# baker-laboratory/NA-MPNN

Hardware: AMD Instinct MI355X
Metric: residues/sec (enc+dec fwd), N~1000 K=48 h=128; seq-recovery vs CPU ref (higher is better)
Workload: dtype f32; 1 GPU; cfg2: B=1 x N=1000 residues per rank, K=48, H=128, 3 enc + 3 dec layers, per-edge GEMMs fp32, seeded random-init weights, independent complexes per rank; precision=fp32, global_batch=1, seq_len=1000, parallelism=replicas x1

## Files before the change

### na_mpnn_amd/csrc/namp.hip

```cpp
#include "../../include/namp.h"
#include "namp_kernels.h"
#include <atomic>
#include "namp_bf16s32.h"
#include "namp_bf16p.h"
#include "namp_node_w.h"
#include "namp_order.h"
#include "namp_attach.h"

#include <cstdarg>
#include <cstdlib>
#include <cstring>
#include <initializer_list>
#include <cstdio>
#include <mutex>
#include <vector>

namespace {

thread_local char g_err[512] = "";

int fail(int code, const char* fmt, ...) {
  va_list ap;
  va_start(ap, fmt);
  vsnprintf(g_err, sizeof(g_err), fmt, ap);
// ... 321 lines not shown
  if (nproj < 0 || nproj > 8 || (nproj > 0 && !proj)) return fail(NAMP_EINVAL, "%s: nproj=%d must be in [0,8]", fn, nproj);
  for (int i = 0; i < nproj; ++i) {
    if (!proj[i].img || !proj[i].out) return fail(NAMP_EINVAL, "%s: proj[%d] has a null image / output", fn, i);
    if (!aligned16(proj[i].img) || !aligned16(proj[i].out) || !aligned16(proj[i].bias) || !aligned16(proj[i].tok))
      return fail(NAMP_EINVAL, "%s: proj[%d] pointers must be 16-byte aligned", fn, i);
    if (proj[i].tok && !S) return fail(NAMP_EINVAL, "%s: proj[%d].tok given but S is null", fn, i);
  }
  return NAMP_OK;
}

struct Out16Req { __bf16* p[8]; int n; bool honoured; };
thread_local Out16Req* g_out16 = nullptr;
thread_local bool g_residue_x1 = false;

int launch_node_linear(const float* X, const int32_t* S, int G_out, int G_src, int N,
                       const NampProj* proj, int nproj, const NampProj* pre, hipStream_t s, bool x3 = false, unsigned* zero = nullptr) {
  NodeLinearArgs a;
  a.X = X; a.S = S; a.G_out = G_out; a.G_src = G_src; a.N = N; a.nproj = nproj; a.zero = zero;
  a.pre.img = pre ? pre->img : nullptr; a.pre.bias = pre ? pre->bias : nullptr;
  a.pre.tok = nullptr; a.pre.out = pre ? pre->out : nullptr;
  for (int i = 0; i < 8; ++i) {
    const NampProj& p = proj[i < nproj ? i : 0];
    a.p[i].img = p.img; a.p[i].bias = p.bias; a.p[i].tok = p.tok; a.p[i].out = p.out;
    a.out16[i] = (g_out16 && i < nproj && i < g_out16->n) ? g_out16->p[i] : nullptr;
    if (a.out16[i]) a.p[i].out = nullptr;
  }
  if (g_out16) g_out16->honoured = true;
  const int units = ((G_out + 15) / 16) * nproj;
  if (x3 && G_out >= 4096 && (g_bf16p.load(std::memory_order_relaxed) & 8) && ensure_attributes() == NAMP_OK) {
    if (g_residue_x1) hipLaunchKernelGGL(node_linear_w_kernel<2>, dim3((G_out + NODEW_ROWS - 1) / NODEW_ROWS), dim3(NODEW_THREADS), NODEW_LDS, s, a);
    else hipLaunchKernelGGL(node_linear_w_kernel<1>, dim3((G_out + NODEW_ROWS - 1) / NODEW_ROWS), dim3(NODEW_THREADS), NODEW_LDS, s, a);
    return NAMP_OK;
  }
  if (x3 && g_residue_x1) hipLaunchKernelGGL(node_linear_kernel<2>, dim3((units + 3) / 4), dim3(256), 0, s, a);
  else if (x3) hipLaunchKernelGGL(node_linear_kernel<1>, dim3((units + 3) / 4), dim3(256), 0, s, a);
  else hipLaunchKernelGGL(node_linear_kernel<0>, dim3((units + 3) / 4), dim3(256), 0, s, a);
  return NAMP_OK;
}

int launch_node_update(const float* ln1_g, const float* ln1_b, const float* Win_img, const float* b_in,
                       const float* Wout_img, const float* b_out, const float* ln2_g, const float* ln2_b,
                       const float* hV, const float* partial, const float* m3_img, const float* m3_b, const int32_t* mask,
                       float* hV_out, const NampProj* proj, int nproj, const int32_t* S, int G, int TPN, hipStream_t s,
                       bool x3 = false) {
  int rc = ensure_attributes();
  if (rc) return rc;
  NodeUpdateArgs a;
  fill_tail(a.t, ln1_g, ln1_b, Win_img, b_in, Wout_img, b_out, ln2_g, ln2_b, hV, mask, hV_out, proj, nproj, S);
  a.t.m3_img = partial ? m3_img : nullptr; a.t.m3_b = m3_b;
  a.partial = partial; a.G = G; a.TPN = TPN;
  const bool multi = x3 || G >= 32 * 2 * device_cus();
  for (int i = 0; i < 8; ++i) {
    a.out16[i] = (multi && g_out16 && i < nproj && i < g_out16->n) ? g_out16->p[i] : nullptr;
    if (a.out16[i]) a.t.p[i].out = nullptr;
  }
  if (multi && g_out16) g_out16->honoured = true;
  if (x3 && g_residue_x1 && a.t.m3_img && !a.t.head_w && nproj <= 4 && G >= 2048 && (g_bf16p.load(std::memory_order_relaxed) & 8))
    hipLaunchKernelGGL(node_update_w_kernel<false>, dim3((G + NODEW_ROWS - 1) / NODEW_ROWS), dim3(NODEW_THREADS), NODEW_LDS, s, a);
  else if (x3 && !g_residue_x1 && a.t.m3_img && !a.t.head_w && nproj <= 4 && G >= 2048 && (g_bf16p.load(std::memory_order_relaxed) & 8))
    hipLaunchKernelGGL(node_update_w_kernel<true>, dim3((G + NODEW_ROWS - 1) / NODEW_ROWS), dim3(NODEW_THREADS), NODEW_LDS, s, a);
  else if (x3 && g_residue_x1)
    hipLaunchKernelGGL((node_update_multi_kernel<2, 2>), dim3((G + 31) / 32), dim3(512), NODE_MULTI_LDS_X3(2), s, a);
  else if (x3)
    hipLaunchKernelGGL((node_update_multi_kernel<2, 1>), dim3((G + 31) / 32), dim3(512), NODE_MULTI_LDS_X3(2), s, a);
  else if (G >= 32 * 2 * device_cus())
    hipLaunchKernelGGL((node_update_multi_kernel<2, 0>), dim3((G + 31) / 32), dim3(512), NODE_MULTI_LDS(2), s, a);
// ... 1756 lines not shown
```

### na_mpnn_amd/csrc/namp_kernels.h

```cpp
#pragma once
#include "namp_device.h"
#ifndef NAMP_MAX_LAYERS
#define NAMP_MAX_LAYERS 8
#endif

static __global__ void pack_image_kernel(const float* __restrict__ W, int ld, int col0, int OUT, int IN,
                                  float* __restrict__ img) {
  const int total = OUT * IN;
  for (int e = blockIdx.x * blockDim.x + threadIdx.x; e < total; e += gridDim.x * blockDim.x) {
    const int r = e & 3, lane = (e >> 2) & 63, t = e >> 8;
    const int ntn = OUT >> 4;
    const int tn = t % ntn, tk = t / ntn;
    const int n = 16 * tn + (lane & 15), k = 16 * tk + 4 * (lane >> 4) + r;
    img[e] = W[(size_t)n * ld + col0 + k];
  }
}

static __global__ void pack_image_bf16_kernel(const float* __restrict__ W, int ld, int col0, __bf16* __restrict__ img) {
  const int e = blockIdx.x * blockDim.x + threadIdx.x;
  if (e >= 128 * 128) return;
  const int j = e & 7, lane = (e >> 3) & 63, tn = (e >> 9) & 7, s = e >> 12;
  const int n = 16 * tn + (lane & 15), k = 32 * s + 16 * (j >> 2) + 4 * (lane >> 4) + (j & 3);
  img[e] = (__bf16)W[(size_t)n * ld + col0 + k];
}
// ... 109 lines not shown
    out[e] = (c < C1) ? nbrs[row * C1 + c] : nodes[((row / NK) * N + idx[row]) * C2 + (c - C1)];
  }
}

struct ProjDesc {
  const float* img;
  const float* bias;
  const float* tok;
  float* out;
};

struct NodeTail {
  const float* hV;
  const int32_t* mask;
  const float* ln1_g; const float* ln1_b;
  const float* Win_img;
  const float* b_in;
  const float* Wout_img;
  const float* b_out;
  const float* ln2_g; const float* ln2_b;
  float* hV_out;
  const int32_t* S;
  const float* m3_img;
  const float* m3_b;
  const float* head_w;
  const float* head_b;
  float* log_probs;
  float* logits;
  int vocab;
  int nproj;
  ProjDesc p[8];
};

__device__ __forceinline__ void tail_head_row(const NodeTail& a, const float* ybase, const int sc, const int orow,
                                              const int lane) {
  float z = -INFINITY;
  if (lane < a.vocab) {
    const float* w = a.head_w + (long)lane * NAMP_H;
    float s0 = 0.f, s1 = 0.f, s2 = 0.f, s3 = 0.f;
#pragma unroll 8
    for (int c = 0; c < NAMP_H; c += 4) {
      const f4 wv = *(const f4*)(w + c);
      s0 = fmaf(wv.x, ybase[(c + 0) * sc], s0); s1 = fmaf(wv.y, ybase[(c + 1) * sc], s1);
      s2 = fmaf(wv.z, ybase[(c + 2) * sc], s2); s3 = fmaf(wv.w, ybase[(c + 3) * sc], s3);
    }
    z = (s0 + s1) + (s2 + s3) + a.head_b[lane];
  }
  float mx = z;
#pragma unroll
  for (int o = 1; o < 64; o <<= 1) mx = fmaxf(mx, __shfl_xor(mx, o));
  float e = (lane < a.vocab) ? expf(z - mx) : 0.f;
#pragma unroll
  for (int o = 1; o < 64; o <<= 1) e += __shfl_xor(e, o);
  if (lane < a.vocab) {
    a.log_probs[(long)orow * a.vocab + lane] = (z - mx) - logf(e);
    if (a.logits) a.logits[(long)orow * a.vocab + lane] = z;
  }
}

#define FFN_LD 132
#define NODE_TAIL_LDS ((16 + 16 + 8 * 16) * FFN_LD * 4)

template <bool DEEP>
__device__ __forceinline__ void node_tail(const NodeTail& a, f4 (&x)[8], const float wsum_m, const int row0, const int nrows, const int G,
                                          float* lds, const int tid, const int wave, const int nwaves, const int lane) {
  float* xs = lds;
// ... 251 lines not shown
    f4 v = c0[nb] + c1[nb];
#pragma unroll
    for (int c = 0; c < 4; ++c) { v[c] += __shfl_xor(v[c], 16); v[c] += __shfl_xor(v[c], 32); }
    o[nb] = v;
  }
}

#define TAIL4_AHEAD 3
template <class FragFn>
__device__ __forceinline__ void tail4_request1(f4 (&wf)[8], const int u, const int lane, FragFn frag) {
#pragma unroll
  for (int tk = 0; tk < 8; ++tk) wf[tk] = frag(u, tk)[lane];
}
template <class FragFn>
__device__ __forceinline__ void tail4_request(f4 (&wf)[TAIL4_AHEAD][8], const int u0, const int total, const int step, const int lane, FragFn frag) {
#pragma unroll
  for (int t = 0; t < TAIL4_AHEAD; ++t) {
    const int u = u0 + t * step;
    tail4_request1(wf[t], u < total ? u : u0, lane, frag);
  }
}
template <class FragFn, class BodyFn, class NextFn>
__device__ __forceinline__ void tail4_phase(f4 (&wf)[TAIL4_AHEAD][8], const int u0, const int total, const int step, const int lane, FragFn frag,
                                            BodyFn body, NextFn next) {
#pragma unroll
  for (int t = 0; t < TAIL4_AHEAD; ++t) {
    const int u = u0 + t * step;
    if (u < total) body(u, wf[t]);
    next(t);
  }
  tail_units<false>(u0 + TAIL4_AHEAD * step, total, step, lane, frag, body);
}

template <int R, typename RowFn, bool SC1, bool M3, bool PF, bool AH>
__device__ __forceinline__ void node_tail_mfma4(const NodeTail& a, f4 (&x)[8], const float wsum_m, const RowFn orow, float* lds,
                                                const int tid, const int wave, const int nwaves, const int lane) {
  static_assert(R == 4 || R == 8, "node_tail_mfma4: 4 or 8 rows");
  constexpr int NB = R / 4;
  constexpr bool AHEAD = AH && !PF && R == 4;
  float* xB = lds;
  float* hB = xB + 128 * R;
  float* oP = hB + 512 * R;
  float* yT = oP + 4 * 128 * R;
  float* red = yT + 128 * R;
  float* yB = red + 64;
  const int m = lane & 15, g = lane >> 4;
  const int cb = (lane >> 2) & 3, j = lane & 3;
  const bool st_lane = lane < 16;
  const auto win_frag = [&](const int u, const int tk) { return (const f4*)a.Win_img + (tk * 32 + u) * 64; };
  const auto wout_frag = [&](const int u, const int tk) { return (const f4*)a.Wout_img + ((8 * (u >> 3) + tk) * 8 + (u & 7)) * 64; };

  f4 wa[AHEAD ? TAIL4_AHEAD : 1][8];
  float bin_a[TAIL4_AHEAD] = {0.f, 0.f, 0.f};
  if constexpr (AHEAD) {
    tail4_request(wa, wave, 32, nwaves, lane, win_frag);
#pragma unroll
    for (int t = 0; t < TAIL4_AHEAD; ++t) {
      const int u = wave + t * nwaves;
      bin_a[t] = a.b_in[16 * (u < 32 ? u : wave) + 4 * cb + g];
    }
  }
  if (M3 && a.m3_img) {
    if (wave == 0 && m < R) {
#pragma unroll
      for (int t = 0; t < 8; ++t) *(f4*)(xB + (m >> 2) * 512 + t * 64 + g * 16 + (m & 3) * 4) = x[t];
      if (g == 0) red[m] = wsum_m;
    }
    __syncthreads();
    {
      f4 xr[NB][8];
      tail4_x<NB>(xr, xB, lane);
      tail_units<PF>(wave, 8, nwaves, lane,
                     [&](const int u, const int tk) { return (const f4*)a.m3_img + (tk * 8 + u) * 64; },
                     [&](const int u, const f4 (&wf)[8]) {
                       f4 o[NB];
                       tail4_unit<NB>(o, wf, xr);
                       if (st_lane) {
                         const f4 b = *(const f4*)(a.m3_b + 16 * u + 4 * cb);
#pragma unroll
                         for (int nb = 0; nb < NB; ++nb) *(f4*)(oP + (4 * nb + j) * NAMP_H + 16 * u + 4 * cb) = o[nb] + b * red[4 * nb + j];
                       }
                     });
    }
    __syncthreads();
    const int mr = m < R ? m : 0;
    int hr = orow(mr);
    if (hr < 0) hr = orow(0) < 0 ? 0 : orow(0);
    const float* hsrc = a.hV + (long)hr * NAMP_H + 4 * g;
#pragma unroll
    for (int t = 0; t < 8; ++t) x[t] = *(const f4*)(hsrc + 16 * t) + *(const f4*)(oP + mr * NAMP_H + 16 * t + 4 * g);
  }

  layernorm_row_T(x, a.ln1_g, a.ln1_b, g);
  if (wave == 0 && m < R) {
#pragma unroll
    for (int t = 0; t < 8; ++t) *(f4*)(xB + (m >> 2) * 512 + t * 64 + g * 16 + (m & 3) * 4) = x[t];
  }
  __syncthreads();
  {
    f4 xr[NB][8];
    tail4_x<NB>(xr, xB, lane);
    const auto body = [&](const int u, const f4 (&wf)[8]) {
      f4 o[NB];
      tail4_unit<NB>(o, wf, xr);
      const int t_ = AHEAD ? (u - wave) / nwaves : 0;
      const float b = (AHEAD && t_ < TAIL4_AHEAD) ? (t_ == 0 ? bin_a[0] : t_ == 1 ? bin_a[1] : bin_a[2]) : a.b_in[16 * u + 4 * cb + g];
#pragma unroll
      for (int nb = 0; nb < NB; ++nb) {
        const float v = g == 0 ? o[nb].x : g == 1 ? o[nb].y : g == 2 ? o[nb].z : o[nb].w;
        hB[((u >> 3) * NB + nb) * 512 + (u & 7) * 64 + cb * 16 + j * 4 + g] = gelu_erf(v + b);
      }
    };
    if constexpr (AHEAD)
      tail4_phase(wa, wave, 32, nwaves, lane, win_frag, body, [&](const int t) {
        const int u = wave + t * nwaves;
        tail4_request1(wa[t], u < 32 ? u : wave, lane, wout_frag);
      });
    else tail_units<PF>(wave, 32, nwaves, lane, win_frag, body);
  }
  __syncthreads();
  {
    const auto body = [&](const int u, const f4 (&wf)[8]) {
      const int tn = u & 7, q = u >> 3;
      f4 xr[NB][8];
      tail4_x<NB>(xr, hB + q * NB * 512, lane);
      f4 o[NB];
      tail4_unit<NB>(o, wf, xr);
      if (st_lane) {
#pragma unroll
        for (int nb = 0; nb < NB; ++nb) *(f4*)(oP + (q * R + 4 * nb + j) * NAMP_H + 16 * tn + 4 * cb) = o[nb];
      }
    };
    if constexpr (AHEAD)
      tail4_phase(wa, wave, 32, nwaves, lane, wout_frag, body, [&](const int pi) {
        if (pi < a.nproj) {
          const int tn = ((wave - pi * 8) % nwaves + nwaves) % nwaves;
          const f4* img = (const f4*)(pi == 0 ? a.p[0].img : pi == 1 ? a.p[1].img : a.p[2].img) + ((tn < 8 ? tn : 0)) * 64 + lane;
#pragma unroll
          for (int tk = 0; tk < 8; ++tk) wa[pi][tk] = img[tk * 8 * 64];
        }
      });
    else tail_units<PF>(wave, 32, nwaves, lane, wout_frag, body);
  }
  __syncthreads();
  const int n_ = tid >> 7, c_ = tid & 127;
  const bool ln_thr = tid < 128 * R;
  const int boff = ln_thr ? (n_ >> 2) * 512 + tail4_off(c_, n_ & 3) : 0;
  float v = 0.f;
  if (ln_thr) {
    v = xB[boff] + a.b_out[c_];
#pragma unroll
    for (int q = 0; q < 4; ++q) v += oP[(q * R + n_) * NAMP_H + c_];
    float s = v;
#pragma unroll
    for (int o = 1; o < 64; o <<= 1) s += __shfl_xor(s, o);
    if (lane == 0) red[wave] = s;
  }
  __syncthreads();
  float d = 0.f;
  if (ln_thr) {
    const float mean = (red[2 * n_] + red[2 * n_ + 1]) * (1.0f / 128.0f);
    d = v - mean;
    float q = d * d;
#pragma unroll
    for (int o = 1; o < 64; o <<= 1) q += __shfl_xor(q, o);
    if (lane == 0) red[32 + wave] = q;
  }
  __syncthreads();
  if (ln_thr) {
    const float rstd = rsqrtf((red[32 + 2 * n_] + red[32 + 2 * n_ + 1]) * (1.0f / 128.0f) + 1e-5f);
    const int orw = orow(n_);
    const float mk = (a.mask && orw >= 0) ? (float)a.mask[orw] : 1.0f;
    const float y = (d * rstd * a.ln2_g[c_] + a.ln2_b[c_]) * mk;
    yT[c_ * R + n_] = y;
    yB[boff] = y;
    if (orw >= 0) st_out<SC1>(a.hV_out + (long)orw * NAMP_H + c_, y);
  }
  if (a.nproj == 0 && !a.head_w) return;
  __syncthreads();
  if (a.head_w) {
    for (int n = wave; n < R; n += nwaves) {
      const int orw = orow(n);
      if (orw >= 0) tail_head_row(a, yT + n, R, orw, lane);
    }
  }
  f4 xr[NB][8];
  tail4_x<NB>(xr, yB, lane);
  int orw[NB];
#pragma unroll
  for (int nb = 0; nb < NB; ++nb) orw[nb] = orow(4 * nb + j);
  auto proj_out = [&](const f4 (&o)[NB], const float* bias, const float* tok, float* out, const int tn) {
    if (!st_lane) return;
    const int c = 16 * tn + 4 * cb;
    const f4 b = bias ? *(const f4*)(bias + c) : (f4){0.f, 0.f, 0.f, 0.f};
#pragma unroll
    for (int nb = 0; nb < NB; ++nb) {
      if (orw[nb] < 0) continue;
      f4 r = o[nb] + b;
      if (tok) r += *(const f4*)(tok + (long)a.S[orw[nb]] * NAMP_H + c);
      float* dst = out + (long)orw[nb] * NAMP_H + c;
      if (SC1) { st_out<true>(dst, r.x); st_out<true>(dst + 1, r.y); st_out<true>(dst + 2, r.z); st_out<true>(dst + 3, r.w); }
      else *(f4*)dst = r;
    }
  };
  if constexpr (PF) {
    tail_units<true>(wave, 8 * (a.nproj < 2 ? a.nproj : 2), nwaves, lane,
                     [&](const int v, const int tk) { return (const f4*)((v >> 3) ? a.p[1].img : a.p[0].img) + (tk * 8 + (v & 7)) * 64; },
                     [&](const int v, const f4 (&wf)[8]) {
                       const bool second = (v >> 3) != 0;
                       f4 o[NB];
                       tail4_unit<NB>(o, wf, xr);
                       proj_out(o, second ? a.p[1].bias : a.p[0].bias, second ? a.p[1].tok : a.p[0].tok, second ? a.p[1].out : a.p[0].out, v & 7);
                     });
    return;
  }
#pragma unroll
  for (int pi = 0; pi < 8; ++pi) {
    if (pi >= a.nproj) break;
    const ProjDesc pd = a.p[pi];
    bool first = AHEAD && pi < TAIL4_AHEAD;
#pragma unroll 1
    for (int tn = ((wave - pi * 8) % nwaves + nwaves) % nwaves; tn < 8; tn += nwaves) {
      f4 o[NB];
      if (first) {
        tail4_unit<NB>(o, wa[pi < TAIL4_AHEAD ? pi : 0], xr);
      } else {
        f4 wf[8];
#pragma unroll
        for (int tk = 0; tk < 8; ++tk) wf[tk] = ((const f4*)pd.img)[(tk * 8 + tn) * 64 + lane];
        tail4_unit<NB>(o, wf, xr);
      }
      first = false;
      proj_out(o, pd.bias, pd.tok, pd.out, tn);
    }
  }
}

template <int R, typename RowFn, bool SC1 = false, bool M3 = true, bool PF = false, bool AH = false>
__device__ __forceinline__ void node_tail_rows(const NodeTail& a, f4 (&x)[8], const float wsum_m, const RowFn orow, float* lds,
                                               const int tid, const int wave, const int nwaves, const int lane) {
#ifndef NAMP_TAIL_VALU
  node_tail_mfma4<R, RowFn, SC1, M3, PF, AH>(a, x, wsum_m, orow, lds, tid, wave, nwaves, lane);
  return;
#endif
  float* xT = lds;
  float* hT = xT + 128 * R;
  float* oP = hT + 512 * R;
  float* yT = oP + 4 * 128 * R;
  float* red = yT + 128 * R;
  const int m = lane & 15, g = lane >> 4;

  if (M3 && a.m3_img) {
    if (wave == 0 && m < R) {
#pragma unroll
      for (int t = 0; t < 8; ++t) {
        xT[(16 * t + 4 * g + 0) * R + m] = x[t].x; xT[(16 * t + 4 * g + 1) * R + m] = x[t].y;
        xT[(16 * t + 4 * g + 2) * R + m] = x[t].z; xT[(16 * t + 4 * g + 3) * R + m] = x[t].w;
      }
      if (g == 0) red[m] = wsum_m;
    }
    __syncthreads();
#pragma unroll 1
    for (int tn = wave; tn < 8; tn += nwaves) {
      f4 wf[8];
#pragma unroll
      for (int tk = 0; tk < 8; ++tk) wf[tk] = ((const f4*)a.m3_img)[(tk * 8 + tn) * 64 + lane];
      float acc[R];
#pragma unroll
      for (int n = 0; n < R; ++n) acc[n] = 0.f;
      rows_fma<R>(acc, wf, xT, g);
#pragma unroll
      for (int n = 0; n < R; ++n) acc[n] = xg_sum(acc[n]);
      if (g == 0) {
        const float b = a.m3_b[16 * tn + m];
#pragma unroll
// ... 285 lines not shown
}

struct EdgeArgs {
  const float* hE;
  float* hE_out;
  const int32_t* E_idx;
  const int32_t* mask;
  const int32_t* mask_attend;
  const int32_t* rank;
  const float* Pa;
  const float* Pj0;
  const float* Pj1;
  const float* W1_img;
  const float* W2_img;
  const float* W3_img;
  const float* b1;
  const float* b2;
  const float* b3;
  const float* ln_g;
  const float* ln_b;
  const float* ePa; const float* ePj;
  const float* eW1_img; const float* eW2_img; const float* eW3_img;
  const float* eb2; const float* eb3;
  uint32_t drop_thresh, drop_seed; float drop_scale;
  const __bf16* hE16; __bf16* hE16_out;
  const __bf16* Pa16; const __bf16* Pj016; const __bf16* Pj116;
  float* partial;
  NodeTail tail;
  int G;
  int G_enc;
  int N, K, TPN;
};

#define EDGE_TAIL_LDS (2 * NAMP_IMG_BYTES + 12 * NAMP_H * 4 + 64 + 2048)

enum { PRE_NONE = 0, PRE_EMBED = 1, PRE_EDGE = 3 };
enum { PREC_F32 = 0, PREC_BF16 = 1, PREC_X3 = 2 };
template <int MODE, int TAIL, int PREC, int PRE, int PERSIST, class Args>
__device__ __forceinline__ void edge_stage(const Args& a, f4 (&x)[8], char* smem) {
  f4 l2pf0 = (f4){0.f, 0.f, 0.f, 0.f}, l2pf1 = l2pf0;
  constexpr bool BF16 = (PREC == PREC_BF16);
  constexpr bool X3 = (PREC == PREC_X3);
  static_assert(PRE == PRE_NONE || (!BF16 && TAIL != 0 && (MODE == MODE_ENC_MSG || MODE == MODE_DEC_MSG)), "PRE: fp32-class message + tail only");
  constexpr bool FUSE = (PRE == PRE_EDGE);
  constexpr bool MSG = (MODE == MODE_ENC_MSG || MODE == MODE_DEC_MSG);
  constexpr bool M3_LDS = MSG && !BF16 && (TAIL == 4 || TAIL == 8);
  char* buf0 = smem;
  char* buf1 = smem + NAMP_IMG_BYTES;
  const int tid = threadIdx.x;
  const int lane = tid & 63;
  const int wave = __builtin_amdgcn_readfirstlane(tid >> 6);
  const int nwaves = blockDim.x >> 6;

  const int m = lane & 15, g = lane >> 4;
  const int npw = nwaves / a.TPN;
  const int node_l = wave / a.TPN, kt = wave - node_l * a.TPN;
  const int bid = xcd_block_index(blockIdx.x, gridDim.x);
  int node = bid * npw + node_l;
  const bool wave_active = (node_l < npw) && (node < a.G);
  if (!wave_active) node = 0;
  const int b_dec = node / a.N;
  const int i_loc = node - b_dec * a.N;
  const int node_enc = (MODE == MODE_DEC_MSG) ? ((b_dec % (a.G_enc / a.N)) * a.N + i_loc) : node;
  const int k = 16 * kt + m;
  const bool valid = wave_active && (k < a.K);
  const long erow = (long)node_enc * a.K + (valid ? k : 0);

// ... 16 lines not shown
    const int j_loc = a.E_idx[erow];
    const int j = node_enc - i_loc + j_loc;
    const float* pa = a.ePa + (long)node_enc * NAMP_H + 4 * g;
    const float* pj = a.ePj + (long)j * NAMP_H + 4 * g;
#pragma unroll
    for (int t = 0; t < 8; ++t) { acc[t] = *(const f4*)(pa + 16 * t); pjv[t] = *(const f4*)(pj + 16 * t); }
  } else {
    const int j_loc = a.E_idx[erow];
    const float* pj;
    if (MODE == MODE_DEC_MSG) {
      const int j_dec = b_dec * a.N + j_loc;
      const bool bw = a.rank[j_dec] < a.rank[node];
      pj = bw ? (a.Pj0 + (long)j_dec * NAMP_H) : (a.Pj1 + (long)(node_enc - i_loc + j_loc) * NAMP_H);
      w_row = valid ? (1.0f / 30.0f) : 0.f;
    } else {
      const int j = node - i_loc + j_loc;
      pj = a.Pj0 + (long)j * NAMP_H;
      if (MODE == MODE_ENC_MSG) {
        int ma;
        if (a.mask_attend) ma = a.mask_attend[erow];
        else ma = a.mask ? (a.mask[node] * a.mask[j]) : 1;
        w_row = valid ? ((float)ma * (1.0f / 30.0f)) : 0.f;
      }
    }
    const float* pa = a.Pa + (long)node * NAMP_H + 4 * g;
    pj += 4 * g;
#pragma unroll
    for (int t = 0; t < 8; ++t) { acc[t] = *(const f4*)(pa + 16 * t); pjv[t] = *(const f4*)(pj + 16 * t); }
  }

  const f4* w0 = (const f4*)buf0 + lane;
  const f4* w1 = (const f4*)buf1 + lane;

  if (BF16) {
    const bf8* bw = (const bf8*)smem + lane;
    dma_to_lds(smem, a.W1_img, 32, wave, nwaves, lane);
    if (MODE != MODE_EMBED) dma_to_lds(smem + NAMP_BIMG_BYTES, a.W2_img, 32, wave, nwaves, lane);
    if (MODE == MODE_ENC_EDGE) dma_to_lds(smem + 2 * NAMP_BIMG_BYTES, a.W3_img, 32, wave, nwaves, lane);
    wait_dma_and_sync();
    chain_gemm_bf16<false, false>(acc, x, bw);
    if (MODE != MODE_EMBED) {
#pragma unroll
      for (int t = 0; t < 8; ++t) acc[t] += pjv[t];
      if (MSG) {
#pragma unroll
        for (int t = 0; t < 8; ++t) { const float b = a.b2[16 * t + m]; y[t] = (f4){b, b, b, b}; }
        chain_gemm_bf16<true, true>(y, acc, bw + (NAMP_BIMG_BYTES / 16));
      } else {
#pragma unroll
        for (int t = 0; t < 8; ++t) y[t] = *(const f4*)(a.b2 + 16 * t + 4 * g);
        chain_gemm_bf16<false, true>(y, acc, bw + (NAMP_BIMG_BYTES / 16));
      }
    }
  } else {
  float* cstf = (float*)(smem + 2 * NAMP_IMG_BYTES + 12 * NAMP_H * 4 + 64);
  if (FUSE) {
    dma_to_lds(buf1, a.eW1_img, 64, wave, nwaves, lane);
    dma_to_lds(buf0, a.eW2_img, 64, wave, nwaves, lane);
    for (int i = tid; i < 512; i += (int)blockDim.x) {
      const float* srcv = i < 128 ? a.eb2 : i < 256 ? a.eb3 : i < 384 ? a.ln_g : a.ln_b;
      cstf[i] = srcv[i & 127];
    }
    wait_dma_and_sync();
    gemm128<X3, false, false>(acc, x, w1);
#pragma unroll
    for (int t = 0; t < 8; ++t) acc[t] += pjv[t];
    __syncthreads();
    dma_to_lds(buf1, a.eW3_img, 64, wave, nwaves, lane);
#pragma unroll
    for (int t = 0; t < 8; ++t) pjv[t] = *(const f4*)(cstf + 16 * t + 4 * g);
    gemm128<X3, false, true>(pjv, acc, w0);
    wait_dma_and_sync();
    dma_to_lds(buf0, a.W1_img, 64, wave, nwaves, lane);
#pragma unroll
    for (int t = 0; t < 8; ++t) acc[t] = *(const f4*)(cstf + 128 + 16 * t + 4 * g);
    gemm128<X3, false, true>(acc, pjv, w1);
#pragma unroll
    for (int t = 0; t < 8; ++t) x[t] += acc[t];
    layernorm_row_T(x, cstf + 256, cstf + 384, g);
    if (valid && (PERSIST == 0 || a.hE_out != nullptr)) {
      float* dst = a.hE_out + erow * NAMP_H + 4 * g;
#pragma unroll
      for (int t = 0; t < 8; ++t) *(f4*)(dst + 16 * t) = x[t];
    }
  }
  if (PRE != PRE_NONE) {
    if (PRE == PRE_EMBED) {
      dma_to_lds(buf1, a.eW1_img, 64, wave, nwaves, lane);
      dma_to_lds(buf0, a.W1_img, 64, wave, nwaves, lane);
#pragma unroll
      for (int t = 0; t < 8; ++t) acc[t] = *(const f4*)(a.eb2 + 16 * t + 4 * g);
      wait_dma_and_sync();
      gemm128<X3, false, false>(acc, x, w1);
#pragma unroll
      for (int t = 0; t < 8; ++t) x[t] = acc[t];
      if (valid && (PERSIST == 0 || a.hE_out != nullptr)) {
        float* dst = a.hE_out + erow * NAMP_H + 4 * g;
#pragma unroll
        for (int t = 0; t < 8; ++t) *(f4*)(dst + 16 * t) = x[t];
      }
    }
    {
      const int j_loc = a.E_idx[erow];
      const float* pj;
      if (MODE == MODE_DEC_MSG) {
        const int j_dec = b_dec * a.N + j_loc;
        const bool bw = a.rank[j_dec] < a.rank[node];
        pj = bw ? (a.Pj0 + (long)j_dec * NAMP_H) : (a.Pj1 + (long)(node_enc - i_loc + j_loc) * NAMP_H);
        w_row = valid ? (1.0f / 30.0f) : 0.f;
      } else {
        const int j = node - i_loc + j_loc;
        pj = a.Pj0 + (long)j * NAMP_H;
        int ma;
        if (a.mask_attend) ma = a.mask_attend[erow];
        else ma = a.mask ? (a.mask[node] * a.mask[j]) : 1;
        w_row = valid ? ((float)ma * (1.0f / 30.0f)) : 0.f;
      }
      const float* pa = a.Pa + (long)node * NAMP_H + 4 * g;
      pj += 4 * g;
#pragma unroll
      for (int t = 0; t < 8; ++t) { acc[t] = *(const f4*)(pa + 16 * t); pjv[t] = *(const f4*)(pj + 16 * t); }
    }
    if (PRE == PRE_EMBED) __syncthreads();
    else wait_dma_and_sync();
    dma_to_lds(buf1, a.W2_img, 64, wave, nwaves, lane);
  } else {
  dma_to_lds(buf0, a.W1_img, 64, wave, nwaves, lane);
  if (MODE != MODE_EMBED) dma_to_lds(buf1, a.W2_img, 64, wave, nwaves, lane);
  wait_dma_and_sync();
  }
  gemm128<X3, false, false>(acc, x, w0);

  if (MODE != MODE_EMBED) {
#pragma unroll
  for (int t = 0; t < 8; ++t) acc[t] += pjv[t];
  if (MSG) {
    if (PRE != PRE_NONE) wait_dma_and_sync();
    else if (M3_LDS) __syncthreads();
    if (M3_LDS) dma_to_lds(buf0, a.W3_img, 64, wave, nwaves, lane);
    if (TAIL == 4 || TAIL == 8) {
      const int slice = (blockIdx.x >> 3) & 31;
      const f4* p0; const f4* p1;
      if (wave < 8) {
        p0 = (const f4*)a.tail.Win_img + (slice * 8 + wave) * 64; p1 = (const f4*)a.tail.Wout_img + (slice * 8 + wave) * 64;
      } else {
        const int q = wave - 8;
        const float* img = q == 0 ? a.tail.p[0].img : q == 1 ? a.tail.p[1].img : q == 2 ? a.tail.p[2].img : a.tail.p[3].img;
        if (q >= a.tail.nproj) img = a.tail.Win_img;
        p0 = (const f4*)img + (slice * 2) * 64; p1 = p0 + 64;
      }
      l2pf0 = p0[lane]; l2pf1 = p1[lane];
    }
#pragma unroll
    for (int t = 0; t < 8; ++t) { const float b = a.b2[16 * t + m]; y[t] = (f4){b, b, b, b}; }
    gemm128<X3, true, true>(y, acc, w1);
  } else {
  if (PRE != PRE_NONE) wait_dma_and_sync();
  else __syncthreads();
  dma_to_lds(buf0, a.W3_img, 64, wave, nwaves, lane);

#pragma unroll
  for (int t = 0; t < 8; ++t) y[t] = *(const f4*)(a.b2 + 16 * t + 4 * g);
  gemm128<X3, false, true>(y, acc, w1);
  wait_dma_and_sync();
  }
  }
  }
  if (MODE == MODE_EMBED) {
    if (valid) {
      if (a.hE16_out) {
        __bf16* dst = a.hE16_out + erow * NAMP_H;
#pragma unroll
        for (int t = 0; t < 8; ++t) st_frag4(dst, t, g, acc[t]);
      } else {
        float* dst = a.hE_out + erow * NAMP_H + 4 * g;
#pragma unroll
        for (int t = 0; t < 8; ++t) *(f4*)(dst + 16 * t) = acc[t];
      }
    }
    return;
  }

  if (MODE == MODE_ENC_EDGE) {
#pragma unroll
    for (int t = 0; t < 8; ++t) acc[t] = *(const f4*)(a.b3 + 16 * t + 4 * g);
    if (BF16) chain_gemm_bf16<false, true>(acc, y, (const bf8*)smem + lane + 2 * (NAMP_BIMG_BYTES / 16));
    else      gemm128<X3, false, true>(acc, y, w0);
// ... 35 lines not shown
    } else {
      float* dpart = (float*)(smem + 2 * NAMP_IMG_BYTES);
      float* dws = dpart + 12 * NAMP_H;
#pragma unroll
      for (int t = 0; t < 8; ++t) {
        const f4 v = gelu_prec<PREC>(y[t]);
        float s = (v.x * wr[0] + v.y * wr[1]) + (v.z * wr[2] + v.w * wr[3]);
        s = xg_sum(s);
        if (g == 0) dpart[wave * NAMP_H + 16 * t + m] = s;
      }
      if (lane == 0) dws[wave] = wsum;
      asm volatile("" :: "v"(l2pf0), "v"(l2pf1));
      if (M3_LDS) wait_dma_and_sync();
      else __syncthreads();
      const int row0 = bid * npw;
      const int trow = row0 + m;
      const bool tvalid = (m < npw) && (trow < a.G);
      const int mm = tvalid ? m : 0;
      float wsum_m = 0.f;
#pragma unroll
      for (int t = 0; t < 8; ++t) y[t] = (f4){0.f, 0.f, 0.f, 0.f};
      for (int q = 0; q < a.TPN; ++q) {
        const float* dp = dpart + (mm * a.TPN + q) * NAMP_H + 4 * g;
#pragma unroll
        for (int t = 0; t < 8; ++t) y[t] += *(const f4*)(dp + 16 * t);
        wsum_m += dws[mm * a.TPN + q];
      }
      if (TAIL == 4 || TAIL == 8) {
        constexpr int R = (TAIL == 4 || TAIL == 8) ? TAIL : 4;
        const ConsecutiveRows orow = {row0, npw, a.G};
        if (M3_LDS) {
          __syncthreads();
          for (int tn = wave; tn < 8; tn += nwaves) {
            const f4 o = tile_gemm1<X3>(*(const f4*)(a.tail.m3_b + 16 * tn + 4 * g) * wsum_m, y, w0, tn);
            if (m < 8) *(f4*)(dpart + m * NAMP_H + 16 * tn + 4 * g) = o;
          }
          __syncthreads();
          const float* hsrc = a.tail.hV + (long)(row0 + mm) * NAMP_H + 4 * g;
          const float* dsrc = dpart + (mm & 7) * NAMP_H + 4 * g;
#pragma unroll
          for (int t = 0; t < 8; ++t) y[t] = *(const f4*)(hsrc + 16 * t) + *(const f4*)(dsrc + 16 * t);
          node_tail_rows<R, ConsecutiveRows, (PERSIST != 0), false, false, !BF16>(a.tail, y, 0.f, orow, (float*)smem, tid, wave, nwaves, lane);
        } else {
          node_tail_rows<R, ConsecutiveRows, (PERSIST != 0), true, false, !BF16>(a.tail, y, wsum_m, orow, (float*)smem, tid, wave, nwaves, lane);
        }
      } else {
        node_tail<false>(a.tail, y, wsum_m, row0, npw, a.G, (float*)smem, tid, wave, nwaves, lane);
      }
    }
  }
}

template <int MODE, int TAIL, int PREC = PREC_F32, int PRE = PRE_NONE>
__global__ __launch_bounds__(768) void edge_mlp_kernel(const EdgeArgs a) {
  extern __shared__ __attribute__((aligned(16))) char smem[];
  f4 x[8];
  edge_stage<MODE, TAIL, PREC, PRE, 0>(a, x, smem);
}

#define NAMP_PERSIST_MAX_STAGES 16
#define NAMP_SYNC_GROUPS 8
#define NAMP_SYNC_WORDS 64
#define NAMP_SYNC_TOP 8
#define NAMP_SYNC_GEN 16
#define NAMP_SYNC_TIMEOUT 32
#define NAMP_SYNC_DEFER 40
#define NAMP_SPIN_LIMIT (1u << 22)

typedef __attribute__((address_space(1))) unsigned int gu32;

__device__ __forceinline__ bool spin_until_ge(gu32* word, unsigned target, gu32* tmo, unsigned code) {
  unsigned spins = 0;
  while (__hip_atomic_load(word, __ATOMIC_RELAXED, __HIP_MEMORY_SCOPE_AGENT) < target) {
    __builtin_amdgcn_s_sleep(2);
    if (++spins > NAMP_SPIN_LIMIT) {
      __hip_atomic_store(tmo, code, __ATOMIC_RELAXED, __HIP_MEMORY_SCOPE_AGENT);
      return false;
// ... 1010 lines not shown
#pragma unroll
    for (int t = 0; t < 8; ++t) acc[t] = a.pre.bias ? *(const f4*)(a.pre.bias + 16 * t + 4 * g) : (f4){0.f, 0.f, 0.f, 0.f};
    if constexpr (X3) chain_gemm_global_x3<X3 == 2>(acc, x, (const bf8*)a.pre.img + lane);
    else chain_gemm_global<8, 8, false>(acc, x, (const f4*)a.pre.img + lane, 8);
    if (pi == 0 && valid && a.pre.out) {
      float* dst = a.pre.out + (long)row * NAMP_H + 4 * g;
#pragma unroll
      for (int t = 0; t < 8; ++t) *(f4*)(dst + 16 * t) = acc[t];
    }
#pragma unroll
    for (int t = 0; t < 8; ++t) x[t] = acc[t];
  }
#pragma unroll
  for (int t = 0; t < 8; ++t) acc[t] = d.bias ? *(const f4*)(d.bias + 16 * t + 4 * g) : (f4){0.f, 0.f, 0.f, 0.f};
  if constexpr (X3) chain_gemm_global_x3<X3 == 2>(acc, x, (const bf8*)d.img + lane);
  else chain_gemm_global<8, 8, false>(acc, x, (const f4*)d.img + lane, 8);
  if (d.tok) {
    const float* tk = d.tok + (long)a.S[rr] * NAMP_H + 4 * g;
#pragma unroll
    for (int t = 0; t < 8; ++t) acc[t] += *(const f4*)(tk + 16 * t);
  }
  if (valid && d.out) {
    float* dst = d.out + (long)row * NAMP_H + 4 * g;
#pragma unroll
    for (int t = 0; t < 8; ++t) *(f4*)(dst + 16 * t) = acc[t];
  }
  if (valid && o16) {
    __bf16* dst = o16 + (long)row * NAMP_H;
#pragma unroll
    for (int t = 0; t < 8; ++t) st_frag4(dst, t, g, acc[t]);
  }
}

struct NodeUpdateArgs {
  NodeTail t;
  const float* partial;
  int G, TPN;
  __bf16* out16[8];
};

static __global__ __launch_bounds__(512) void node_update_kernel(const NodeUpdateArgs a) {
  extern __shared__ __attribute__((aligned(16))) char smem[];
  const int tid = threadIdx.x, lane = tid & 63;
  const int wave = __builtin_amdgcn_readfirstlane(tid >> 6);
  const int m = lane & 15, g = lane >> 4;
  const int row0 = blockIdx.x * 16;
  const int rr = (row0 + m < a.G) ? row0 + m : row0;
  f4 x[8];
  float wsum_m = 0.f;
  if (a.t.m3_img) {
#pragma unroll
    for (int t = 0; t < 8; ++t) x[t] = (f4){0.f, 0.f, 0.f, 0.f};
    for (int p = 0; p < a.TPN; ++p) wsum_m += a.partial[(long)a.G * a.TPN * NAMP_H + (long)rr * a.TPN + p];
  } else {
    const float* src = a.t.hV + (long)rr * NAMP_H + 4 * g;
#pragma unroll
    for (int t = 0; t < 8; ++t) x[t] = *(const f4*)(src + 16 * t);
  }
  if (a.partial) {
    for (int p = 0; p < a.TPN; ++p) {
      const float* ps_ = a.partial + ((long)rr * a.TPN + p) * NAMP_H + 4 * g;
#pragma unroll
      for (int t = 0; t < 8; ++t) x[t] += *(const f4*)(ps_ + 16 * t);
    }
  }
  node_tail<true>(a.t, x, wsum_m, row0, 16, a.G, (float*)smem, tid, wave, 8, lane);
// ... 1028 lines not shown
```

Measured before the change: 2.074 million residues/s.

## Add per-tile node linear kernel and stage tail operand vectors in LDS

```diff
diff --git a/na_mpnn_amd/csrc/namp.hip b/na_mpnn_amd/csrc/namp.hip
--- a/na_mpnn_amd/csrc/namp.hip
+++ b/na_mpnn_amd/csrc/namp.hip
@@ -377,6 +377,13 @@
     else hipLaunchKernelGGL(node_linear_w_kernel<1>, dim3((G_out + NODEW_ROWS - 1) / NODEW_ROWS), dim3(NODEW_THREADS), NODEW_LDS, s, a);
     return NAMP_OK;
   }
+  const int ntiles = (G_out + 15) / 16;
+  if (nproj >= 1 && nproj <= NODE_LINEAR_TILE_MAXPROJ && ntiles <= device_cus()) {
+    if (x3 && g_residue_x1) hipLaunchKernelGGL(node_linear_tile_kernel<2>, dim3(ntiles), dim3(512), 0, s, a);
+    else if (x3) hipLaunchKernelGGL(node_linear_tile_kernel<1>, dim3(ntiles), dim3(512), 0, s, a);
+    else hipLaunchKernelGGL(node_linear_tile_kernel<0>, dim3(ntiles), dim3(512), 0, s, a);
+    return NAMP_OK;
+  }
   if (x3 && g_residue_x1) hipLaunchKernelGGL(node_linear_kernel<2>, dim3((units + 3) / 4), dim3(256), 0, s, a);
   else if (x3) hipLaunchKernelGGL(node_linear_kernel<1>, dim3((units + 3) / 4), dim3(256), 0, s, a);
   else hipLaunchKernelGGL(node_linear_kernel<0>, dim3((units + 3) / 4), dim3(256), 0, s, a);
diff --git a/na_mpnn_amd/csrc/namp_kernels.h b/na_mpnn_amd/csrc/namp_kernels.h
--- a/na_mpnn_amd/csrc/namp_kernels.h
+++ b/na_mpnn_amd/csrc/namp_kernels.h
@@ -165,6 +165,8 @@
   ProjDesc p[8];
 };
 
+enum { TOP_LN1G = 0, TOP_LN1B = 1, TOP_BIN = 2, TOP_BOUT = 6, TOP_LN2G = 7, TOP_LN2B = 8, TOP_M3B = 9, TOP_B2 = 10, TOP_PBIAS = 11, TOP_N = 19 };
+
 __device__ __forceinline__ void tail_head_row(const NodeTail& a, const float* ybase, const int sc, const int orow,
                                               const int lane) {
   float z = -INFINITY;
@@ -482,10 +484,17 @@
   tail_units<false>(u0 + TAIL4_AHEAD * step, total, step, lane, frag, body);
 }
 
-template <int R, typename RowFn, bool SC1, bool M3, bool PF, bool AH>
+template <int R, typename RowFn, bool SC1, bool M3, bool PF, bool AH, bool OPS = false>
 __device__ __forceinline__ void node_tail_mfma4(const NodeTail& a, f4 (&x)[8], const float wsum_m, const RowFn orow, float* lds,
-                                                const int tid, const int wave, const int nwaves, const int lane) {
+                                                const int tid, const int wave, const int nwaves, const int lane, const float* ops = nullptr) {
   static_assert(R == 4 || R == 8, "node_tail_mfma4: 4 or 8 rows");
+  const float* const ln1_g = OPS ? ops + TOP_LN1G * 128 : a.ln1_g;
+  const float* const ln1_b = OPS ? ops + TOP_LN1B * 128 : a.ln1_b;
+  const float* const b_in = OPS ? ops + TOP_BIN * 128 : a.b_in;
+  const float* const b_out = OPS ? ops + TOP_BOUT * 128 : a.b_out;
+  const float* const ln2_g = OPS ? ops + TOP_LN2G * 128 : a.ln2_g;
+  const float* const ln2_b = OPS ? ops + TOP_LN2B * 128 : a.ln2_b;
+  const float* const m3_b = OPS ? ops + TOP_M3B * 128 : a.m3_b;
   constexpr int NB = R / 4;
   constexpr bool AHEAD = AH && !PF && R == 4;
   float* xB = lds;
@@ -507,7 +516,7 @@
 #pragma unroll
     for (int t = 0; t < TAIL4_AHEAD; ++t) {
       const int u = wave + t * nwaves;
-      bin_a[t] = a.b_in[16 * (u < 32 ? u : wave) + 4 * cb + g];
+      bin_a[t] = b_in[16 * (u < 32 ? u : wave) + 4 * cb + g];
     }
   }
   if (M3 && a.m3_img) {
@@ -526,7 +535,7 @@
                        f4 o[NB];
                        tail4_unit<NB>(o, wf, xr);
                        if (st_lane) {
-                         const f4 b = *(const f4*)(a.m3_b + 16 * u + 4 * cb);
+                         const f4 b = *(const f4*)(m3_b + 16 * u + 4 * cb);
 #pragma unroll
                          for (int nb = 0; nb < NB; ++nb) *(f4*)(oP + (4 * nb + j) * NAMP_H + 16 * u + 4 * cb) = o[nb] + b * red[4 * nb + j];
                        }
@@ -541,7 +550,7 @@
     for (int t = 0; t < 8; ++t) x[t] = *(const f4*)(hsrc + 16 * t) + *(const f4*)(oP + mr * NAMP_H + 16 * t + 4 * g);
   }
 
-  layernorm_row_T(x, a.ln1_g, a.ln1_b, g);
+  layernorm_row_T(x, ln1_g, ln1_b, g);
   if (wave == 0 && m < R) {
 #pragma unroll
     for (int t = 0; t < 8; ++t) *(f4*)(xB + (m >> 2) * 512 + t * 64 + g * 16 + (m & 3) * 4) = x[t];
@@ -554,7 +563,7 @@
       f4 o[NB];
       tail4_unit<NB>(o, wf, xr);
       const int t_ = AHEAD ? (u - wave) / nwaves : 0;
-      const float b = (AHEAD && t_ < TAIL4_AHEAD) ? (t_ == 0 ? bin_a[0] : t_ == 1 ? bin_a[1] : bin_a[2]) : a.b_in[16 * u + 4 * cb + g];
+      const float b = (AHEAD && t_ < TAIL4_AHEAD) ? (t_ == 0 ? bin_a[0] : t_ == 1 ? bin_a[1] : bin_a[2]) : b_in[16 * u + 4 * cb + g];
 #pragma unroll
       for (int nb = 0; nb < NB; ++nb) {
         const float v = g == 0 ? o[nb].x : g == 1 ? o[nb].y : g == 2 ? o[nb].z : o[nb].w;
@@ -598,7 +607,7 @@
   const int boff = ln_thr ? (n_ >> 2) * 512 + tail4_off(c_, n_ & 3) : 0;
   float v = 0.f;
   if (ln_thr) {
-    v = xB[boff] + a.b_out[c_];
+    v = xB[boff] + b_out[c_];
 #pragma unroll
     for (int q = 0; q < 4; ++q) v += oP[(q * R + n_) * NAMP_H + c_];
     float s = v;
@@ -621,7 +630,7 @@
     const float rstd = rsqrtf((red[32 + 2 * n_] + red[32 + 2 * n_ + 1]) * (1.0f / 128.0f) + 1e-5f);
     const int orw = orow(n_);
     const float mk = (a.mask && orw >= 0) ? (float)a.mask[orw] : 1.0f;
-    const float y = (d * rstd * a.ln2_g[c_] + a.ln2_b[c_]) * mk;
+    const float y = (d * rstd * ln2_g[c_] + ln2_b[c_]) * mk;
     yT[c_ * R + n_] = y;
     yB[boff] = y;
     if (orw >= 0) st_out<SC1>(a.hV_out + (long)orw * NAMP_H + c_, y);
@@ -681,16 +690,16 @@
         tail4_unit<NB>(o, wf, xr);
       }
       first = false;
-      proj_out(o, pd.bias, pd.tok, pd.out, tn);
-    }
-  }
-}
-
-template <int R, typename RowFn, bool SC1 = false, bool M3 = true, bool PF = false, bool AH = false>
+      proj_out(o, (OPS && pd.bias) ? ops + (TOP_PBIAS + pi) * 128 : pd.bias, pd.tok, pd.out, tn);
+    }
+  }
+}
+
+template <int R, typename RowFn, bool SC1 = false, bool M3 = true, bool PF = false, bool AH = false, bool OPS = false>
 __device__ __forceinline__ void node_tail_rows(const NodeTail& a, f4 (&x)[8], const float wsum_m, const RowFn orow, float* lds,
-                                               const int tid, const int wave, const int nwaves, const int lane) {
+                                               const int tid, const int wave, const int nwaves, const int lane, const float* ops = nullptr) {
 #ifndef NAMP_TAIL_VALU
-  node_tail_mfma4<R, RowFn, SC1, M3, PF, AH>(a, x, wsum_m, orow, lds, tid, wave, nwaves, lane);
+  node_tail_mfma4<R, RowFn, SC1, M3, PF, AH, OPS>(a, x, wsum_m, orow, lds, tid, wave, nwaves, lane, ops);
   return;
 #endif
   float* xT = lds;
@@ -1042,7 +1051,29 @@
   int N, K, TPN;
 };
 
-#define EDGE_TAIL_LDS (2 * NAMP_IMG_BYTES + 12 * NAMP_H * 4 + 64 + 2048)
+#define EDGE_CST_OFF (2 * NAMP_IMG_BYTES + 12 * NAMP_H * 4 + 64)
+#define EDGE_OPS_OFF (EDGE_CST_OFF + 2048)
+#define EDGE_TAIL_LDS (EDGE_OPS_OFF + TOP_N * NAMP_H * 4)
+static_assert(EDGE_TAIL_LDS <= 160 * 1024, "the fused edge stages need more LDS than a CU has");
+static_assert(TOP_PBIAS + 8 == TOP_N, "one bias row per projection descriptor (NodeTail.p[8])");
+#define TOP_ROUNDS 3
+static_assert(TOP_ROUNDS * 7 >= TOP_N, "every vector of the tail-operand block needs a wave");
+
+template <class Args>
+__device__ __forceinline__ const float* tail_operand_vector(const Args& a, const int v) {
+  const float* p = nullptr;
+  if (v == TOP_LN1G) p = a.tail.ln1_g;
+  if (v == TOP_LN1B) p = a.tail.ln1_b;
+  if (v >= TOP_BIN && v < TOP_BIN + 4 && a.tail.b_in) p = a.tail.b_in + (v - TOP_BIN) * NAMP_H;
+  if (v == TOP_BOUT) p = a.tail.b_out;
+  if (v == TOP_LN2G) p = a.tail.ln2_g;
+  if (v == TOP_LN2B) p = a.tail.ln2_b;
+  if (v == TOP_M3B) p = a.tail.m3_b;
+  if (v == TOP_B2) p = a.b2;
+#pragma unroll
+  for (int q = 0; q < 8; ++q) if (v == TOP_PBIAS + q && q < a.tail.nproj) p = a.tail.p[q].bias;
+  return p;
+}
 
 enum { PRE_NONE = 0, PRE_EMBED = 1, PRE_EDGE = 3 };
 enum { PREC_F32 = 0, PREC_BF16 = 1, PREC_X3 = 2 };
@@ -1125,6 +1156,36 @@
   const f4* w0 = (const f4*)buf0 + lane;
   const f4* w1 = (const f4*)buf1 + lane;
 
+  constexpr bool OPS = !BF16 && (TAIL == 4 || TAIL == 8);
+  float* ops = (float*)(smem + EDGE_OPS_OFF);
+  f2 opv[TOP_ROUNDS];
+  if constexpr (OPS) {
+#pragma unroll
+    for (int r = 0; r < TOP_ROUNDS; ++r) {
+      const float* p = tail_operand_vector(a, wave + r * nwaves);
+      opv[r] = p ? *(const f2*)(p + 2 * lane) : (f2){0.f, 0.f};
+    }
+  }
+  float* cstf = (float*)(smem + EDGE_CST_OFF);
+  f2 cv = (f2){0.f, 0.f};
+  if constexpr (FUSE) {
+    if (wave < 4) cv = *(const f2*)((wave == 0 ? a.eb2 : wave == 1 ? a.eb3 : wave == 2 ? a.ln_g : a.ln_b) + 2 * lane);
+  }
+  const auto wait_dma_ops_and_sync = [&]() {
+    asm volatile("s_waitcnt vmcnt(0)" ::: "memory");
+    if constexpr (OPS) {
+#pragma unroll
+      for (int r = 0; r < TOP_ROUNDS; ++r) {
+        const int v = wave + r * nwaves;
+        if (v < TOP_N) *(f2*)(ops + v * NAMP_H + 2 * lane) = opv[r];
+      }
+    }
+    if constexpr (FUSE) {
+      if (wave < 4) *(f2*)(cstf + wave * NAMP_H + 2 * lane) = cv;
+    }
+    __syncthreads();
+  };
+
   if (BF16) {
     const bf8* bw = (const bf8*)smem + lane;
     dma_to_lds(smem, a.W1_img, 32, wave, nwaves, lane);
@@ -1146,15 +1207,10 @@
       }
     }
   } else {
-  float* cstf = (float*)(smem + 2 * NAMP_IMG_BYTES + 12 * NAMP_H * 4 + 64);
   if (FUSE) {
     dma_to_lds(buf1, a.eW1_img, 64, wave, nwaves, lane);
     dma_to_lds(buf0, a.eW2_img, 64, wave, nwaves, lane);
-    for (int i = tid; i < 512; i += (int)blockDim.x) {
-      const float* srcv = i < 128 ? a.eb2 : i < 256 ? a.eb3 : i < 384 ? a.ln_g : a.ln_b;
-      cstf[i] = srcv[i & 127];
-    }
-    wait_dma_and_sync();
+    wait_dma_ops_and_sync();
     gemm128<X3, false, false>(acc, x, w1);
 #pragma unroll
     for (int t = 0; t < 8; ++t) acc[t] += pjv[t];
@@ -1183,7 +1239,7 @@
       dma_to_lds(buf0, a.W1_img, 64, wave, nwaves, lane);
 #pragma unroll
       for (int t = 0; t < 8; ++t) acc[t] = *(const f4*)(a.eb2 + 16 * t + 4 * g);
-      wait_dma_and_sync();
+      wait_dma_ops_and_sync();
       gemm128<X3, false, false>(acc, x, w1);
 #pragma unroll
       for (int t = 0; t < 8; ++t) x[t] = acc[t];
@@ -1220,7 +1276,7 @@
   } else {
   dma_to_lds(buf0, a.W1_img, 64, wave, nwaves, lane);
   if (MODE != MODE_EMBED) dma_to_lds(buf1, a.W2_img, 64, wave, nwaves, lane);
-  wait_dma_and_sync();
+  wait_dma_ops_and_sync();
   }
   gemm128<X3, false, false>(acc, x, w0);
 
@@ -1244,8 +1300,9 @@
       }
       l2pf0 = p0[lane]; l2pf1 = p1[lane];
     }
-#pragma unroll
-    for (int t = 0; t < 8; ++t) { const float b = a.b2[16 * t + m]; y[t] = (f4){b, b, b, b}; }
+    const float* b2v = OPS ? ops + TOP_B2 * NAMP_H : a.b2;
+#pragma unroll
+    for (int t = 0; t < 8; ++t) { const float b = b2v[16 * t + m]; y[t] = (f4){b, b, b, b}; }
     gemm128<X3, true, true>(y, acc, w1);
   } else {
   if (PRE != PRE_NONE) wait_dma_and_sync();
@@ -1347,7 +1404,7 @@
         if (M3_LDS) {
           __syncthreads();
           for (int tn = wave; tn < 8; tn += nwaves) {
-            const f4 o = tile_gemm1<X3>(*(const f4*)(a.tail.m3_b + 16 * tn + 4 * g) * wsum_m, y, w0, tn);
+            const f4 o = tile_gemm1<X3>(*(const f4*)((OPS ? ops + TOP_M3B * NAMP_H : a.tail.m3_b) + 16 * tn + 4 * g) * wsum_m, y, w0, tn);
             if (m < 8) *(f4*)(dpart + m * NAMP_H + 16 * tn + 4 * g) = o;
           }
           __syncthreads();
@@ -1355,9 +1412,9 @@
           const float* dsrc = dpart + (mm & 7) * NAMP_H + 4 * g;
 #pragma unroll
           for (int t = 0; t < 8; ++t) y[t] = *(const f4*)(hsrc + 16 * t) + *(const f4*)(dsrc + 16 * t);
-          node_tail_rows<R, ConsecutiveRows, (PERSIST != 0), false, false, !BF16>(a.tail, y, 0.f, orow, (float*)smem, tid, wave, nwaves, lane);
+          node_tail_rows<R, ConsecutiveRows, (PERSIST != 0), false, false, !BF16, OPS>(a.tail, y, 0.f, orow, (float*)smem, tid, wave, nwaves, lane, ops);
         } else {
-          node_tail_rows<R, ConsecutiveRows, (PERSIST != 0), true, false, !BF16>(a.tail, y, wsum_m, orow, (float*)smem, tid, wave, nwaves, lane);
+          node_tail_rows<R, ConsecutiveRows, (PERSIST != 0), true, false, !BF16, OPS>(a.tail, y, wsum_m, orow, (float*)smem, tid, wave, nwaves, lane, ops);
         }
       } else {
         node_tail<false>(a.tail, y, wsum_m, row0, npw, a.G, (float*)smem, tid, wave, nwaves, lane);
@@ -2434,6 +2491,113 @@
   }
 }
 
+template <int X3>
+__device__ __forceinline__ void tile_frags_request(f4 (&wf)[8], const float* img, const int tn, const int lane) {
+  if constexpr (X3) {
+    const f4* w = (const f4*)img + lane;
+#pragma unroll
+    for (int s = 0; s < 4; ++s) {
+      wf[s] = w[(s * 8 + tn) * 64];
+      wf[4 + s] = X3 == 2 ? wf[s] : w[NAMP_BIMG_BYTES / 16 + (s * 8 + tn) * 64];
+    }
+  } else {
+    const f4* w = (const f4*)img + lane;
+#pragma unroll
+    for (int tk = 0; tk < 8; ++tk) wf[tk] = w[(tk * 8 + tn) * 64];
+  }
+}
+template <int X3>
+__device__ __forceinline__ f4 tile_frags_gemm(f4 acc, const f4 (&x)[8], const f4 (&wf)[8]) {
+  if constexpr (X3) {
+#pragma unroll
+    for (int s = 0; s < 4; ++s) {
+      bf8 hi, mid;
+      if constexpr (X3 == 2) { hi = pack_bf16<false>(x[2 * s], x[2 * s + 1]); mid = hi; }
+      else split_x3(x[2 * s], x[2 * s + 1], hi, mid);
+      acc = mfma_xs<X3 == 2>(__builtin_bit_cast(bf8, wf[s]), __builtin_bit_cast(bf8, wf[4 + s]), hi, mid, acc);
+    }
+  } else {
+#pragma unroll
+    for (int tk = 0; tk < 8; ++tk) {
+#pragma unroll
+      for (int r = 0; r < 4; ++r) acc = mfma4(wf[tk][r], x[tk][r], acc);
+    }
+  }
+  return acc;
+}
+
+#define NODE_LINEAR_TILE_MAXPROJ 2
+template <int X3>
+__global__ __launch_bounds__(512) void node_linear_tile_kernel(const NodeLinearArgs a) {
+  __shared__ __attribute__((aligned(16))) float hs[16 * FFN_LD];
+  const int lane = threadIdx.x & 63;
+  const int wave = __builtin_amdgcn_readfirstlane(threadIdx.x >> 6);
+  if (a.zero && blockIdx.x == 0 && threadIdx.x < 64) a.zero[threadIdx.x] = 0u;
+  const int m = lane & 15, g = lane >> 4;
+  const int row = blockIdx.x * 16 + m;
+  const bool valid = row < a.G_out;
+  const int rr = valid ? row : 0;
+  const int b = rr / a.N;
+  const int src_row = (b % (a.G_src / a.N)) * a.N + (rr - b * a.N);
+  const int col = 16 * wave + 4 * g;
+  const f4 zero4 = (f4){0.f, 0.f, 0.f, 0.f};
+
+  f4 x[8];
+  const float* src = a.X + (long)src_row * NAMP_H + 4 * g;
+#pragma unroll
+  for (int t = 0; t < 8; ++t) x[t] = *(const f4*)(src + 16 * t);
+  bool any_tok = false;
+#pragma unroll
+  for (int q = 0; q < NODE_LINEAR_TILE_MAXPROJ; ++q) any_tok |= q < a.nproj && a.p[q].tok != nullptr;
+  const int tok_row = any_tok ? a.S[rr] : 0;
+
+  auto request = [&](const int q, f4 (&wf)[8], f4& bias, f4& tk) {
+    tile_frags_request<X3>(wf, a.p[q].img, wave, lane);
+    bias = a.p[q].bias ? *(const f4*)(a.p[q].bias + col) : zero4;
+    tk = a.p[q].tok ? *(const f4*)(a.p[q].tok + (long)tok_row * NAMP_H + col) : zero4;
+  };
+  auto store = [&](const int q, const f4 acc) {
+    if (valid && a.p[q].out) *(f4*)(a.p[q].out + (long)row * NAMP_H + col) = acc;
+    if (valid && a.out16[q]) st_frag4(a.out16[q] + (long)row * NAMP_H, wave, g, acc);
+  };
+
+  f4 cur[8], nxt[8], cb, nb, ct, nt, h = zero4;
+  if (a.pre.img) {
+    f4 pf[8];
+    tile_frags_request<X3>(pf, a.pre.img, wave, lane);
+    h = a.pre.bias ? *(const f4*)(a.pre.bias + col) : zero4;
+    request(0, cur, cb, ct);
+    __builtin_amdgcn_sched_barrier(0);
+    h = tile_frags_gemm<X3>(h, x, pf);
+    *(f4*)(hs + m * FFN_LD + col) = h;
+    __syncthreads();
+#pragma unroll
+    for (int t = 0; t < 8; ++t) x[t] = *(const f4*)(hs + m * FFN_LD + 16 * t + 4 * g);
+  } else {
+    request(0, cur, cb, ct);
+  }
+  f4 prev = zero4;
+#pragma unroll
+  for (int pi = 0; pi < NODE_LINEAR_TILE_MAXPROJ; ++pi) {
+    if (pi >= a.nproj) break;
+    const bool more = pi + 1 < NODE_LINEAR_TILE_MAXPROJ && pi + 1 < a.nproj;
+    if (more) request(pi + 1 < NODE_LINEAR_TILE_MAXPROJ ? pi + 1 : 0, nxt, nb, nt);
+    if (pi == 0) { if (a.pre.img && valid && a.pre.out) *(f4*)(a.pre.out + (long)row * NAMP_H + col) = h; }
+    else store(pi - 1, prev);
+    __builtin_amdgcn_sched_barrier(0);
+    f4 acc = tile_frags_gemm<X3>(cb, x, cur);
+    if (a.p[pi].tok) acc += ct;
+    if (!more) store(pi, acc);
+    prev = acc;
+    __builtin_amdgcn_sched_barrier(0);
+    if (more) {
+#pragma unroll
+      for (int t = 0; t < 8; ++t) cur[t] = nxt[t];
+      cb = nb; ct = nt;
+    }
+  }
+}
+
 struct NodeUpdateArgs {
   NodeTail t;
   const float* partial;
```

Result: faster. 2.130 million residues/s (median of 6 runs) (+2.7%).
